# uni-medical/UniMedVL

Measured on AMD Instinct MI355X. Metric: VQA greedy decode tokens/s, UniMedVL-14B (BAGEL-7B-MoT dims), batch 8 x 448x448 per GPU, higher is better.
Workload: dtype bf16; 1 GPU; configs[1]: UniMedVL-14B bf16 VQA greedy decode, batch=8 448x448, 1xMI355X; batch_per_gpu=8, image=448x448, parallelism=dp1, decode=hipGraph

## Files before the change

include/unimedvl_hip.h:

```cpp
#ifndef UNIMEDVL_HIP_H
#define UNIMEDVL_HIP_H
#include <stddef.h>
#include <stdint.h>

#ifdef __cplusplus
extern "C" {
#endif

typedef void* umv_stream_t;

int umv_version(void);
const char* umv_last_error(void);

size_t umv_packed_weight_elems(int N, int K);
int umv_pack_weight_bf16(const uint16_t* w, uint16_t* packed, int N, int K, umv_stream_t stream);
size_t umv_repacked_weight_elems(int N, int K, int th);
int umv_repack_weight_rows_bf16(const uint16_t* packed16, uint16_t* out, int N, int K, int th, umv_stream_t stream);
int umv_pack_weight_swiglu_bf16(const uint16_t* gate, const uint16_t* up, uint16_t* packed, int I, int K,
                                umv_stream_t stream);

enum {
    UMV_EPI_BIAS = 1,
    UMV_EPI_GELU_TANH = 2,
    UMV_EPI_SILU = 4,
// ... 26 lines not shown
    const int64_t* sample_step;
} umv_gemm_args;
int umv_gemm_bf16(const umv_gemm_args* a, umv_stream_t stream);
int umv_gemm_tile_config(int M, int N, int K);

size_t umv_packed_weight_fp8_bytes(int N, int K);
int umv_quantize_pack_weight_fp8(const uint16_t* w, const uint16_t* w_up, uint8_t* packed8, float* scale, uint16_t* deq,
                                 uint16_t* deq_up, int rows, int K, umv_stream_t stream);
int umv_gemm_fp8w(const umv_gemm_args* a, umv_stream_t stream);

size_t umv_packed_weight_mxfp4_bytes(int N, int K);
int umv_quantize_pack_weight_mxfp4(const uint16_t* w, const uint16_t* w_up, uint8_t* packed4, uint16_t* deq, uint16_t* deq_up,
                                   int rows, int K, umv_stream_t stream);
int umv_gemm_mxfp4w(const umv_gemm_args* a, umv_stream_t stream);
int umv_gemm_mxfp4t(const umv_gemm_args* a, umv_stream_t stream);

size_t umv_packed_weight_fp8_mfma_bytes(int N, int K);
int umv_repack_weight_fp8_mfma(const uint8_t* packed8, uint8_t* out, int N, int K, umv_stream_t stream);
int umv_quantize_act_fp8(const uint16_t* x, int64_t ldx, const int32_t* row_idx, uint8_t* xq, int64_t ldq, float* x_scale,
                         uint16_t* deq, int64_t ldd, int M, int K, umv_stream_t stream);
typedef struct {
    const uint8_t* xq;
    int64_t ldq;
    const float* x_scale;
    const uint8_t* wp;
    const float* w_scale;
    const uint16_t* bias;
    const uint16_t* residual;
    int64_t ldr;
    void* out;
// ... 118 lines not shown
```

unimedvl_amd/_lib.py:

```python
import ctypes as C
import os

HERE = os.path.dirname(os.path.abspath(__file__))
LIB_PATH = os.environ.get("UMV_LIB_PATH") or os.path.join(HERE, "lib", "libunimedvl_hip.so")

EPI_BIAS, EPI_GELU_TANH, EPI_SILU, EPI_RESIDUAL, EPI_SWIGLU, EPI_OUT_F32 = 1, 2, 4, 8, 16, 32


class GemmArgs(C.Structure):
    _fields_ = [
        ("x", C.c_void_p), ("ldx", C.c_int64), ("wp", C.c_void_p), ("bias", C.c_void_p),
        ("residual", C.c_void_p), ("ldr", C.c_int64), ("out", C.c_void_p), ("ldo", C.c_int64),
        ("row_idx", C.c_void_p), ("M", C.c_int), ("N", C.c_int), ("K", C.c_int), ("epilogue", C.c_int),
        ("norm_w", C.c_void_p), ("norm_eps", C.c_float), ("tile_rows", C.c_int), ("w_scale", C.c_void_p),
        ("k_splits", C.c_int), ("split_stride", C.c_int64), ("argmax_partial", C.c_void_p), ("x_rows", C.c_int64),
        ("sample_temperature", C.c_float), ("sample_seed", C.c_uint64), ("sample_step", C.c_void_p),
    ]


class QkvPostArgs(C.Structure):
    _fields_ = [
        ("qkv", C.c_void_p), ("q_out", C.c_void_p), ("k_slab", C.c_void_p), ("vt_slab", C.c_void_p),
        ("k_seg_stride", C.c_int64), ("k_head_stride", C.c_int64), ("v_seg_stride", C.c_int64),
        ("v_head_stride", C.c_int64), ("v_d_stride", C.c_int64),
# ... 44 lines not shown
    "umv_last_error": (C.c_char_p, []),
    "umv_packed_weight_elems": (C.c_size_t, [C.c_int, C.c_int]),
    "umv_pack_weight_bf16": (C.c_int, [C.c_void_p, C.c_void_p, C.c_int, C.c_int, C.c_void_p]),
    "umv_repacked_weight_elems": (C.c_size_t, [C.c_int, C.c_int, C.c_int]),
    "umv_repack_weight_rows_bf16": (C.c_int, [C.c_void_p, C.c_void_p, C.c_int, C.c_int, C.c_int, C.c_void_p]),
    "umv_pack_weight_swiglu_bf16": (C.c_int, [C.c_void_p, C.c_void_p, C.c_void_p, C.c_int, C.c_int, C.c_void_p]),
    "umv_gemm_bf16": (C.c_int, [C.POINTER(GemmArgs), C.c_void_p]),
    "umv_packed_weight_fp8_bytes": (C.c_size_t, [C.c_int, C.c_int]),
    "umv_quantize_pack_weight_fp8": (C.c_int, [C.c_void_p, C.c_void_p, C.c_void_p, C.c_void_p, C.c_void_p, C.c_void_p,
                                               C.c_int, C.c_int, C.c_void_p]),
    "umv_gemm_fp8w": (C.c_int, [C.POINTER(GemmArgs), C.c_void_p]),
    "umv_packed_weight_mxfp4_bytes": (C.c_size_t, [C.c_int, C.c_int]),
    "umv_quantize_pack_weight_mxfp4": (C.c_int, [C.c_void_p, C.c_void_p, C.c_void_p, C.c_void_p, C.c_void_p, C.c_int, C.c_int,
                                                 C.c_void_p]),
    "umv_gemm_mxfp4w": (C.c_int, [C.POINTER(GemmArgs), C.c_void_p]),
    "umv_gemm_mxfp4t": (C.c_int, [C.POINTER(GemmArgs), C.c_void_p]),
    "umv_residual_rmsnorm_bf16": (C.c_int, [C.c_void_p, C.c_int, C.c_int64, C.c_int64, C.c_void_p, C.c_void_p, C.c_void_p, C.c_int,
                                            C.c_int, C.c_float, C.c_void_p]),
    "umv_rmsnorm_bf16": (C.c_int, [C.c_void_p, C.c_void_p, C.c_void_p, C.c_void_p, C.c_void_p, C.c_int, C.c_int,
                                   C.c_float, C.c_void_p]),
    "umv_layernorm_bf16": (C.c_int, [C.c_void_p, C.c_void_p, C.c_void_p, C.c_void_p, C.c_int, C.c_int, C.c_float,
                                     C.c_void_p]),
    "umv_embed_gather_bf16": (C.c_int, [C.c_void_p, C.c_void_p, C.c_void_p, C.c_void_p, C.c_int, C.c_int, C.c_void_p]),
    "umv_add_rows_bf16": (C.c_int, [C.c_void_p, C.c_void_p, C.c_void_p, C.c_void_p, C.c_void_p, C.c_void_p, C.c_int,
                                    C.c_int, C.c_void_p]),
    "umv_argmax_bf16": (C.c_int, [C.c_void_p, C.c_int64, C.c_void_p, C.c_int, C.c_int, C.c_void_p]),
    "umv_sample_bf16": (C.c_int, [C.c_void_p, C.c_int64, C.c_void_p, C.c_int, C.c_int, C.c_float, C.c_uint64, C.c_void_p,
                                  C.c_void_p]),
    "umv_cast_pad_f32_bf16": (C.c_int, [C.c_void_p, C.c_int64, C.c_void_p, C.c_int64, C.c_int, C.c_int, C.c_int,
                                        C.c_void_p]),
# ... 62 lines not shown
```

unimedvl_amd/build.py:

```python
import hashlib
import os
import subprocess
import sys

HERE = os.path.dirname(os.path.abspath(__file__))
CSRC = os.path.join(HERE, "csrc")
LIBDIR = os.path.join(HERE, "lib")
LIB = os.path.join(LIBDIR, "libunimedvl_hip.so")
SOURCES = ["host_error.hip", "elementwise.hip", "pack.hip", "gemm.hip", "gemm_w4.hip", "gemm_fp8mfma.hip", "gemm_mxfp4.hip", "gemm_mxfp4t.hip", "attention.hip", "attention_prefill.hip", "vision.hip"]
FLAGS = ["--offload-arch=gfx950", "-O3", "-std=c++17", "-fPIC", "-ffp-contract=off",
         "-Wno-unused-result", "-fgpu-rdc" if False else "-fno-gpu-rdc"]
FILE_FLAGS = {"attention_prefill.hip": ["-mllvm", "-amdgpu-mfma-vgpr-form"]}
if os.environ.get("UMV_ATTN_TRACE", "0") not in ("0", ""):
    FILE_FLAGS["attention_prefill.hip"] = FILE_FLAGS["attention_prefill.hip"] + ["-DUMV_ATTN_TRACE"]
if os.environ.get("UMV_ATTN_PAIR_DEBUG", "0") not in ("0", ""):
    FILE_FLAGS["attention_prefill.hip"] = FILE_FLAGS["attention_prefill.hip"] + ["-DUMV_ATTN_PAIR_DEBUG=1"]
if os.environ.get("UMV_GEMM_ABLATIONS", "0") not in ("0", ""):
    FILE_FLAGS["gemm_w4.hip"] = ["-DUMV_GEMM_ABLATIONS"]


def _stamp():
    h = hashlib.sha256()
    for f in sorted(os.listdir(CSRC)) + ["../../include/unimedvl_hip.h"]:
        p = os.path.join(CSRC, f)
# ... 59 lines not shown
```

unimedvl_amd/config.py:

```python
import json
import os
from dataclasses import dataclass, field, asdict
from typing import Tuple


@dataclass
class UniMedVLConfig:
    hidden: int = 3584
    layers: int = 28
    heads: int = 28
    kv_heads: int = 4
    inter: int = 18944
    vocab: int = 152064
    rope_theta: float = 1e6
    rms_eps: float = 1e-6
    max_position: int = 32768
    llm_weight_dtype: str = "bf16"
    llm_fp4_keep_bf16: bool = True
    llm_act_dtype: str = "bf16"
    vit_hidden: int = 1152
    vit_layers: int = 26
    vit_heads: int = 16
    vit_inter: int = 4304
    patch: int = 14
    vit_side: int = 70
    ln_eps: float = 1e-6
    max_latent: int = 64
    latent_patch: int = 2
    z_channels: int = 16
    vae_ch: int = 128
    vae_mult: Tuple[int, ...] = (1, 2, 4, 4)
    vae_res: int = 2
    scale_factor: float = 0.3611
# ... 42 lines not shown
```

unimedvl_amd/csrc/gemm_skinny.h:

```cpp
#pragma once
#include "common.h"
#include "../../include/unimedvl_hip.h"
#include "gemm_epilogue.h"
#include "gemm_internal.h"
#include "quant.h"

#define SK_WAVES 8
#define SK_XMAX 16

template <int NT_>
struct SkBf16 {
    static constexpr int NT = NT_, KH = 1;
    struct Unit { bf16x8 w[NT]; };
    int TH, tile_elems;
    bool rowlane;
    const bf16_t* wbase[NT];
    __device__ __forceinline__ SkBf16(const umv_gemm_args& a, int KT, int NTT, int, int nt0, int lane) {
        const int r = lane & 15, g = lane >> 4;
        TH = a.tile_rows > 0 ? a.tile_rows : 16;
        tile_elems = 4 * TH * 8;
        rowlane = r < TH;
#pragma unroll
        for (int t = 0; t < NT; ++t) {
            const bool tv = (nt0 + t) < NTT;
            wbase[t] = a.wp + ((int64_t)(tv ? nt0 + t : 0) * KT) * tile_elems + (g * TH + (rowlane ? r : 0)) * 8;
        }
    }
    __device__ __forceinline__ void load(Unit& b, int kt, bool ok) const {
#pragma unroll
        for (int t = 0; t < NT; ++t)
            b.w[t] = (ok && rowlane) ? __builtin_nontemporal_load(reinterpret_cast<const bf16x8*>(wbase[t] + (int64_t)kt * tile_elems)) : zero_frag();
    }
    __device__ __forceinline__ void frags(const Unit& b, bf16x8 (&wf)[KH][NT]) const {
#pragma unroll
        for (int t = 0; t < NT; ++t) wf[0][t] = b.w[t];
    }
};

template <int NT_>
struct SkE4m3 {
    static constexpr int NT = NT_, KH = 2, TH = 16;
    struct Unit { u32x4 w[NT]; };
    const uint8_t* wbase[NT];
    float wscale[NT];
    __device__ __forceinline__ SkE4m3(const umv_gemm_args& a, int KT8, int NTT, int, int nt0, int lane) {
        const uint8_t* wq = reinterpret_cast<const uint8_t*>(a.wp);
#pragma unroll
        for (int t = 0; t < NT; ++t) {
            const bool tv = (nt0 + t) < NTT;
            const int nt = tv ? nt0 + t : 0;
            wbase[t] = wq + ((int64_t)nt * KT8 * 64 + lane) * 16;
            wscale[t] = a.w_scale[nt * 16 + (lane & 15)];
        }
    }
    __device__ __forceinline__ void load(Unit& b, int kt, bool ok) const {
#pragma unroll
        for (int t = 0; t < NT; ++t)
            b.w[t] = ok ? __builtin_nontemporal_load(reinterpret_cast<const u32x4*>(wbase[t] + (int64_t)kt * 1024)) : (u32x4){0u, 0u, 0u, 0u};
    }
    __device__ __forceinline__ void frags(const Unit& b, bf16x8 (&wf)[KH][NT]) const {
#pragma unroll
        for (int t = 0; t < NT; ++t) cvt_fp8x16(b.w[t], wscale[t], wf[0][t], wf[1][t]);
    }
};

template <int NP>
struct SkMxfp4 {
    static constexpr int NT = 2 * NP, KH = 2, TH = 16;
    struct Unit { u32x4 w[NP]; uint32_t s[NP]; };
    const uint8_t* wbase[NP];
    const uint8_t* sbase[NP];
    __device__ __forceinline__ SkMxfp4(const umv_gemm_args& a, int KT8, int, int NPT, int, int lane) {
        const uint8_t* img = reinterpret_cast<const uint8_t*>(a.wp);
        const uint8_t* scales = img + (int64_t)NPT * KT8 * 1024;
        const int p0 = blockIdx.x * NP;
#pragma unroll
        for (int i = 0; i < NP; ++i) {
            const int p = (p0 + i) < NPT ? p0 + i : 0;
            wbase[i] = img + ((int64_t)p * KT8 * 64 + lane) * 16;
            sbase[i] = scales + ((int64_t)p * KT8 * 16 + (lane & 15)) * 4;
        }
    }
    __device__ __forceinline__ void load(Unit& b, int kt, bool ok) const {
#pragma unroll
        for (int i = 0; i < NP; ++i) {
            b.w[i] = ok ? __builtin_nontemporal_load(reinterpret_cast<const u32x4*>(wbase[i] + (int64_t)kt * 1024)) : (u32x4){0u, 0u, 0u, 0u};
            b.s[i] = ok ? *reinterpret_cast<const uint32_t*>(sbase[i] + (int64_t)kt * 64) : 0x7F7F7F7Fu;
        }
    }
    __device__ __forceinline__ void frags(const Unit& b, bf16x8 (&wf)[KH][NT]) const {
#pragma unroll
        for (int i = 0; i < NP; ++i) {
            const uint32_t s = b.s[i];
            wf[0][2 * i] = cvt_fp4x8(b.w[i].x, e8m0_scale(s & 0xFFu));
            wf[1][2 * i] = cvt_fp4x8(b.w[i].y, e8m0_scale((s >> 8) & 0xFFu));
            wf[0][2 * i + 1] = cvt_fp4x8(b.w[i].z, e8m0_scale((s >> 16) & 0xFFu));
            wf[1][2 * i + 1] = cvt_fp4x8(b.w[i].w, e8m0_scale(s >> 24));
        }
    }
};

template <int NW, int NT, int MB>
__device__ __forceinline__ void skinny16_reduce_epilogue(const umv_gemm_args& a, float* red, const f32x4 (&acc)[NT][MB], int tid,
                                                         int lane, int wave, int nt0, int NTT, int nsplit, int TH) {
    constexpr int E4 = NT * MB;
#pragma unroll
    for (int t = 0; t < NT; ++t)
#pragma unroll
        for (int mb = 0; mb < MB; ++mb) reinterpret_cast<f32x4*>(red)[(wave * E4 + t * MB + mb) * 64 + lane] = acc[t][mb];
    __syncthreads();
    EpiCtx e{a.bias, a.residual, a.ldr, a.out, a.ldo, a.N, a.epilogue};
    if (nsplit > 1) {
// ... 65 lines not shown
    bool xvalid[MB];
#pragma unroll
    for (int mb = 0; mb < MB; ++mb) {
        int m = mb * 16 + r;
        xvalid[mb] = m < a.M;
        int64_t row = xvalid[mb] ? (a.row_idx ? (int64_t)a.row_idx[m] : (int64_t)m) : 0;
        xrow[mb] = a.x + row * a.ldx;
    }
    f32x4 acc[NT][MB];
#pragma unroll
    for (int t = 0; t < NT; ++t)
#pragma unroll
        for (int mb = 0; mb < MB; ++mb) acc[t][mb] = (f32x4){0.f, 0.f, 0.f, 0.f};

    const int nsplit = a.k_splits > 1 ? a.k_splits : 1;
    const int kts = (KT + nsplit - 1) / nsplit;
    const int ks0 = (int)blockIdx.y * kts, ks1 = min(KT, ks0 + kts);
    const int kt_per = (max(0, ks1 - ks0) + SK_WAVES - 1) / SK_WAVES;
    const int kt_begin = ks0 + wave * kt_per;
    const int kt_end = min(ks1, kt_begin + kt_per);
    constexpr int UPL = 2 / KH;
    const int kt_lo = XL != 0 ? (kt_begin & -UPL) : kt_begin;
    const int nk = max(0, kt_end - kt_lo);
    const int nchunks = (nk + U - 1) / U;
    const F f(a, KT, NTT, NPT, nt0, lane);
    static_assert(!XL || ((U * KH) % 2 == 0 && NORM == 0), "full-line x staging: whole lines per chunk, no fused norm");
    static_assert(XL != 1 || MB == 1, "one-piece staging serves one 16-row tile of at most 8 valid rows");
    constexpr int XLN = U * KH / 2, XLP = XL == 1 ? 1 : 2 * MB;
    const int xchunk = (lane & 7) ^ ((lane >> 3) & 7);
    const bf16_t* xprow[XL ? XLP : 1];
    bool xpvalid[XL ? XLP : 1];
    if constexpr (XL != 0) {
#pragma unroll
        for (int q = 0; q < XLP; ++q) {
            const int m = q * 8 + (lane >> 3);
            xpvalid[q] = m < a.M;
            const int64_t row = xpvalid[q] ? (a.row_idx ? (int64_t)a.row_idx[m] : (int64_t)m) : 0;
            xprow[q] = a.x + row * a.ldx + xchunk * 8;
        }
    }
    char* xstage = reinterpret_cast<char*>(red) + wave * (XLN * XLP * 1024);
// ... 106 lines not shown
                const int rr = XL == 1 ? (r & 7) : r;
#pragma unroll
                for (int u = 0; u < U; ++u)
#pragma unroll
                    for (int h = 0; h < KH; ++h)
#pragma unroll
                        for (int mb = 0; mb < MB; ++mb) {
                            const int j = u * KH + h;
                            b.x[u][h][mb] = *reinterpret_cast<const bf16x8*>(xstage + (j >> 1) * (XLP * 1024) + (mb * 16 + rr) * 128 +
                                                                             ((((j & 1) * 4 + g) ^ (rr & 7)) << 4));
                        }
            }
#pragma unroll
            for (int u = 0; u < U; ++u) {
                bf16x8 wf[KH][NT];
                f.frags(b.w[u], wf);
#pragma unroll
                for (int h = 0; h < KH; ++h)
#pragma unroll
                    for (int t = 0; t < NT; ++t)
#pragma unroll
                        for (int mb = 0; mb < MB; ++mb) acc[t][mb] = mfma16(wf[h][t], b.x[u][h][mb], acc[t][mb]);
            }
        }
    };
    for (int c = 0; c < nchunks; c += 2) {
        if (DB && c + 1 < nchunks) load_chunk(c + 1, b1);
        consume(b0, c);
        if (c + 1 < nchunks) {
            if (!DB) load_chunk(c + 1, b1);
            if (c + 2 < nchunks && DB) load_chunk(c + 2, b0);
// ... 42 lines not shown
```

unimedvl_amd/csrc/pack.hip:

```cpp
#include "common.h"
#include "../../include/unimedvl_hip.h"
#include "quant.h"
#include <stdlib.h>

__global__ void pack_weight_kernel(const bf16_t* __restrict__ w, bf16_t* __restrict__ p, int N, int K, int NTT,
                                   int KT, int interleave_I, const bf16_t* __restrict__ w2) {
    int64_t gid = (int64_t)blockIdx.x * blockDim.x + threadIdx.x;
    int64_t total = (int64_t)NTT * KT * 64;
    if (gid >= total) return;
    int lane = (int)(gid & 63);
    int64_t tile = gid >> 6;
    int kt = (int)(tile % KT);
    int nt = (int)(tile / KT);
    int r = lane & 15, g = lane >> 4;
    int k = kt * 32 + g * 8;
    const bf16_t* src = w;
    int n;
    if (interleave_I > 0) {
        int t = nt >> 1;
        n = t * 16 + r;
        src = (nt & 1) ? w2 : w;
        if (n >= interleave_I) n = -1;
    } else {
        n = nt * 16 + r;
// ... 262 lines not shown
                                              uint16_t* deq_up, int rows, int K, umv_stream_t stream) {
    UMV_CHECK(w && packed4 && rows > 0 && K > 0, UMV_ERR_ARG, "quantize_pack_weight_mxfp4: bad args");
    UMV_CHECK((K % 32) == 0 && K <= 65536, UMV_ERR_ARG, "quantize_pack_weight_mxfp4: K (%d) must be a multiple of 32 (the block) and <= 65536",
              K);
    UMV_CHECK(!w_up || (rows % 16) == 0, UMV_ERR_ARG, "quantize_pack_weight_mxfp4: SwiGLU image needs I %% 16 == 0 (I=%d)", rows);
    UMV_CHECK(!(deq_up && !w_up), UMV_ERR_ARG, "quantize_pack_weight_mxfp4: deq_up without w_up");
    UMV_CHECK(((uintptr_t)w | (uintptr_t)w_up | (uintptr_t)deq | (uintptr_t)deq_up | (uintptr_t)packed4) % 16 == 0, UMV_ERR_ARG,
              "quantize_pack_weight_mxfp4: every buffer must be 16-byte aligned");
    const int NTT = (w_up ? 2 : 1) * ((rows + 15) / 16), NP = (NTT + 1) / 2, KT8 = (K + 63) / 64;
    const size_t lds = (size_t)32 * 2 * KT8;
    hipLaunchKernelGGL(quantize_pack_mxfp4_kernel, dim3(NP), dim3(256), lds, (hipStream_t)stream, (const bf16_t*)w, (const bf16_t*)w_up,
                       packed4, (bf16_t*)deq, (bf16_t*)deq_up, rows, K, KT8, NTT, NP);
    UMV_LAUNCH_CHECK();
    return UMV_OK;
}
```

unimedvl_amd/ops.py:

```python
import ctypes as C
import functools

import torch

from . import _lib
from ._lib import (EPI_BIAS, EPI_GELU_TANH, EPI_OUT_F32, EPI_RESIDUAL, EPI_SILU, EPI_SWIGLU, AttnArgs, GemmArgs,
                   QkvPostArgs, check)

BF16 = torch.bfloat16


_raw_stream = getattr(torch._C, "_cuda_getCurrentRawStream", None)


def _stream():
    if _raw_stream is not None:
        return C.c_void_p(_raw_stream(torch.cuda.current_device()))
    return C.c_void_p(torch.cuda.current_stream().cuda_stream)


def on_device(fn):
    @functools.wraps(fn)
    def wrapper(self, *args, **kwargs):
        dev = torch.device(self.device)
# ... 12 lines not shown
    return torch.cuda.device(dev)


def _p(t):
    return None if t is None else C.c_void_p(t.data_ptr())


def _req(t, dtype, name):
    if not t.is_cuda:
        raise _lib.UmvError(f"{name}: tensor must live on the GPU (no CPU fallback)")
    if t.dtype != dtype:
        raise _lib.UmvError(f"{name}: expected {dtype}, got {t.dtype}")
    return t


class PackedLinear:

    __slots__ = ("wp", "bias", "N", "K", "swiglu", "th", "w8", "scale", "w8m", "w4")

    def __init__(self, wp, bias, N, K, swiglu=False, th=16, w8=None, scale=None, w4=None):
        self.wp, self.bias, self.N, self.K, self.swiglu, self.th = wp, bias, N, K, swiglu, th
        self.w8, self.scale = w8, scale
        self.w8m = None
        self.w4 = w4

    def drop_bf16(self):
        if self.w4 is None:
            raise _lib.UmvError("drop_bf16 needs MXFP4 weights (from_weight_mxfp4 / from_gate_up_mxfp4)")
        self.wp = None
        return self

    def enable_fp8_mfma(self, keep_bf16=False):
        if self.w8m is not None:
            if not keep_bf16:
                self.wp = None
            return self
        if self.w8 is None:
            raise _lib.UmvError("enable_fp8_mfma needs fp8 weights (from_weight_fp8 / from_gate_up_fp8)")
        lib = _lib.load()
# ... 94 lines not shown
    @staticmethod
    def from_gate_up(gate, up):
        lib = _lib.load()
        gate = _req(gate.contiguous(), BF16, "gate")
        up = _req(up.contiguous(), BF16, "up")
        I, K = gate.shape
        assert I % 16 == 0, "intermediate size must be a multiple of 16"
        wp = torch.empty(lib.umv_packed_weight_elems(2 * I, K), dtype=BF16, device=gate.device)
        check(lib.umv_pack_weight_swiglu_bf16(_p(gate), _p(up), _p(wp), I, K, _stream()), "umv_pack_weight_swiglu_bf16")
        return PackedLinear(wp, None, 2 * I, K, swiglu=True)

    def nbytes(self):
        return self.wp.numel() * 2 if self.wp is not None else self.w4.numel()


def gemm(x, lin, out=None, *, M=None, residual=None, act=None, row_idx=None, out_f32=False, use_bias=True,
         norm_w=None, norm_eps=1e-6, act8=False, argmax_partial=None, sample=None):
    lib = _lib.load()
    _req(x, BF16, "x")
    assert x.stride(-1) == 1
    M = x.shape[0] if M is None else M
    flags = 0
    if lin.bias is not None and use_bias:
        flags |= EPI_BIAS
    if act == "gelu_tanh":
        flags |= EPI_GELU_TANH
    elif act == "silu":
        flags |= EPI_SILU
    elif act is not None:
        raise ValueError(act)
    if lin.swiglu:
        flags |= EPI_SWIGLU
# ... 66 lines not shown
            row_idx=row_idx.data_ptr() if row_idx is not None else None,
            M=M, N=lin.N, K=lin.K, epilogue=flags, norm_w=None, norm_eps=norm_eps, tile_rows=0,
            w_scale=lin.scale.data_ptr(), argmax_partial=amax, **_sample_fields(sample, amax))
        check(lib.umv_gemm_fp8w(C.byref(a), _stream()), "umv_gemm_fp8w")
        return out
    a = GemmArgs(
        x=x.data_ptr(), ldx=x.stride(0), wp=lin.wp.data_ptr(),
        bias=lin.bias.data_ptr() if (flags & EPI_BIAS) else None,
        residual=residual.data_ptr() if residual is not None else None,
        ldr=residual.stride(0) if residual is not None else 0,
        out=out.data_ptr(), ldo=out.stride(0),
        row_idx=row_idx.data_ptr() if row_idx is not None else None,
        M=M, N=lin.N, K=lin.K, epilogue=flags,
        norm_w=norm_w.data_ptr() if norm_w is not None else None, norm_eps=norm_eps, tile_rows=lin.th, argmax_partial=amax,
        x_rows=x.shape[0], **_sample_fields(sample, amax))
    check(lib.umv_gemm_bf16(C.byref(a), _stream()), "umv_gemm_bf16")
    return out


def rmsnorm(x, w, eps, out=None, w_gen=None, expert=None):
    lib = _lib.load()
    _req(x, BF16, "x")
    T, H = x.shape
    out = torch.empty_like(x) if out is None else out
    check(lib.umv_rmsnorm_bf16(_p(x), _p(w), _p(w_gen), _p(expert), _p(out), T, H, eps, _stream()), "umv_rmsnorm_bf16")
    return out


def layernorm(x, w, b, eps, out=None):
    lib = _lib.load()
# ... 134 lines not shown
          "umv_quantize_act_fp8")
    return out


def _sample_fields(sample, amax):
    if sample is None:
        return {}
    if amax is None:
        raise _lib.UmvError("gemm: sample=(temperature, seed, step) is a mode of the argmax_partial epilogue")
    t, seed, step = sample
    if not float(t) > 0.0:
        raise _lib.UmvError(f"gemm: sampling temperature must be > 0 (got {t})")
    return dict(sample_temperature=float(t), sample_seed=int(seed) & (2 ** 64 - 1), sample_step=None if step is None else step.data_ptr())


def gemm_splitk(x, lin, partials, k_splits, *, M=None):
    lib = _lib.load()
    _req(x, BF16, "x")
    _req(partials, torch.float32, "partials")
    M = x.shape[0] if M is None else M
    assert partials.dim() == 3 and partials.shape[0] == k_splits and partials.shape[2] == lin.N and partials.is_contiguous()
    assert lin.th == 16 and not lin.swiglu
    a = GemmArgs(x=x.data_ptr(), ldx=x.stride(0), wp=None if lin.wp is None else lin.wp.data_ptr(), out=partials.data_ptr(), ldo=lin.N,
                 M=M, N=lin.N, K=lin.K, epilogue=0, tile_rows=0, k_splits=k_splits, split_stride=partials.stride(0))
    if lin.w8 is not None:
        a.wp, a.w_scale = lin.w8.data_ptr(), lin.scale.data_ptr()
        check(lib.umv_gemm_fp8w(C.byref(a), _stream()), "umv_gemm_fp8w")
    elif lin.w4 is not None and M <= 64:
        a.wp = lin.w4.data_ptr()
        check(lib.umv_gemm_mxfp4w(C.byref(a), _stream()), "umv_gemm_mxfp4w")
    elif lin.w4 is not None and lin.wp is None:
        a.wp = lin.w4.data_ptr()
        check(lib.umv_gemm_mxfp4t(C.byref(a), _stream()), "umv_gemm_mxfp4t")
    else:
        check(lib.umv_gemm_bf16(C.byref(a), _stream()), "umv_gemm_bf16")
    return partials


def residual_rmsnorm(partials, seq, w, eps, out):
    lib = _lib.load()
    _req(partials, torch.float32, "partials")
    _req(seq, BF16, "seq")
    S, T, H = partials.shape
    assert seq.shape == (T, H) and seq.is_contiguous() and out.is_contiguous() and partials.is_contiguous()
    check(lib.umv_residual_rmsnorm_bf16(_p(partials), S, partials.stride(0), partials.stride(1), _p(seq), _p(w), _p(out), T, H, eps,
                                        _stream()), "umv_residual_rmsnorm_bf16")
    return out

# ... 115 lines not shown
```

unimedvl_amd/weights.py:

```python
import math

import torch

from . import ops
from .config import UniMedVLConfig

BF16 = torch.bfloat16


class LayerWeights:
    __slots__ = ("qkv", "o", "gate_up", "down", "in_norm", "post_norm", "q_norm", "k_norm")


def _dev(t, device):
    return t.to(device=device, dtype=BF16).contiguous()


class _NoStore:
    @staticmethod
    def linear(key, build):
        return build()

    @staticmethod
    def tensor(name, build):
# ... 37 lines not shown
        self.act8 = cfg.llm_act_dtype == "fp8"
        keep = self.fp4_keep_bf16 = bool(cfg.llm_fp4_keep_bf16) or not fp4
        self.embed = _tensor(get, device, p + "embed_tokens.weight")
        self.und, self.gen = [], []
        for l in range(cfg.layers):
            self.und.append(self._layer(get, device, p + f"layers.{l}.", "", fp8, fp4, keep))
            self.gen.append(self._layer(get, device, p + f"layers.{l}.", "_moe_gen", fp8, fp4, keep) if load_gen else None)
            if self.act8:
                for lw in (self.und[-1], self.gen[-1]):
                    if lw is not None:
                        for lin in (lw.qkv, lw.o, lw.gate_up, lw.down):
                            lin.enable_fp8_mfma()
        self.norm = _tensor(get, device, p + "norm.weight")
        self.norm_gen = _tensor(get, device, p + "norm_moe_gen.weight") if load_gen else None
        self.lm_head = _linear(get, device, "language_model.lm_head.weight", fp8=fp8 or fp4)
        hd = cfg.head_dim
        inv_freq = 1.0 / (cfg.rope_theta ** (torch.arange(0, hd, 2, dtype=torch.int64).float() / hd))
        pos = torch.arange(cfg.max_position, dtype=torch.float32)
        freqs = (inv_freq[None, :, None].float() @ pos[None, None, :]).transpose(1, 2)[0]
        emb = torch.cat((freqs, freqs), dim=-1)
        self.cos = emb.cos().to(BF16).to(device)
        self.sin = emb.sin().to(BF16).to(device)

    @staticmethod
    def _layer(get, device, p, suf, fp8=False, fp4=False, keep_bf16=True):
        lw = LayerWeights()
        a = p + "self_attn."
        st = _store(get)

        def build_qkv():
# ... 8 lines not shown
            u = _dev(get(p + f"mlp{suf}.up_proj.weight"), device)
            if fp4:
                return ops.PackedLinear.from_gate_up_mxfp4(g, u, keep_bf16=keep_bf16)
            return ops.PackedLinear.from_gate_up_fp8(g, u) if fp8 else ops.PackedLinear.from_gate_up(g, u)
        lw.qkv = st.linear(a + f"qkv_proj{suf}", build_qkv)
        lw.o = _linear(get, device, a + f"o_proj{suf}.weight", fp8=fp8, fp4=fp4, keep_bf16=keep_bf16)
        lw.gate_up = st.linear(p + f"mlp{suf}.gate_up_proj", build_gate_up)
        lw.down = _linear(get, device, p + f"mlp{suf}.down_proj.weight", fp8=fp8, fp4=fp4, keep_bf16=keep_bf16)
        lw.in_norm = _tensor(get, device, p + f"input_layernorm{suf}.weight")
        lw.post_norm = _tensor(get, device, p + f"post_attention_layernorm{suf}.weight")
        lw.q_norm = _tensor(get, device, a + f"q_norm{suf}.weight")
        lw.k_norm = _tensor(get, device, a + f"k_norm{suf}.weight")
        return lw

    def decode_weight_bytes(self):
        nb = (lambda lin: lin.w8.numel()) if self.fp8 else (lambda lin: lin.w4.numel()) if self.fp4 else (lambda lin: lin.nbytes())
        n = self.lm_head.w8.numel() if self.fp4 else nb(self.lm_head)
        for lw in self.und:
            n += nb(lw.qkv) + nb(lw.o) + nb(lw.gate_up) + nb(lw.down)
        return n


class ViTLayer:
    __slots__ = ("qkv", "out", "fc1", "fc2", "ln1_w", "ln1_b", "ln2_w", "ln2_b")


class ViTWeights:
    def __init__(self, cfg: UniMedVLConfig, get, device):
        p = "vit_model.vision_model."
        self.k_in = 3 * cfg.patch ** 2
        self.k_pad = (self.k_in + 31) // 32 * 32
# ... 71 lines not shown
```

Baseline: 2550 tokens/s.

## Stream losslessly 13-bit-compressed bf16 weights in decode MLP and lm_head GEMMs

```diff
diff --git a/include/unimedvl_hip.h b/include/unimedvl_hip.h
--- a/include/unimedvl_hip.h
+++ b/include/unimedvl_hip.h
@@ -64,6 +64,10 @@
                                    int rows, int K, umv_stream_t stream);
 int umv_gemm_mxfp4w(const umv_gemm_args* a, umv_stream_t stream);
 int umv_gemm_mxfp4t(const umv_gemm_args* a, umv_stream_t stream);
+
+size_t umv_packed_weight_z13_bytes(int N, int K);
+int umv_pack_weight_z13(const uint16_t* packed16, uint8_t* z13, int N, int K, umv_stream_t stream);
+int umv_gemm_z13w(const umv_gemm_args* a, const void* z13, umv_stream_t stream);
 
 size_t umv_packed_weight_fp8_mfma_bytes(int N, int K);
 int umv_repack_weight_fp8_mfma(const uint8_t* packed8, uint8_t* out, int N, int K, umv_stream_t stream);
diff --git a/unimedvl_amd/_lib.py b/unimedvl_amd/_lib.py
--- a/unimedvl_amd/_lib.py
+++ b/unimedvl_amd/_lib.py
@@ -82,6 +82,9 @@
     "umv_quantize_pack_weight_mxfp4": (C.c_int, [C.c_void_p, C.c_void_p, C.c_void_p, C.c_void_p, C.c_void_p, C.c_int, C.c_int,
                                                  C.c_void_p]),
     "umv_gemm_mxfp4w": (C.c_int, [C.POINTER(GemmArgs), C.c_void_p]),
+    "umv_packed_weight_z13_bytes": (C.c_size_t, [C.c_int, C.c_int]),
+    "umv_pack_weight_z13": (C.c_int, [C.c_void_p, C.c_void_p, C.c_int, C.c_int, C.c_void_p]),
+    "umv_gemm_z13w": (C.c_int, [C.POINTER(GemmArgs), C.c_void_p, C.c_void_p]),
     "umv_gemm_mxfp4t": (C.c_int, [C.POINTER(GemmArgs), C.c_void_p]),
     "umv_residual_rmsnorm_bf16": (C.c_int, [C.c_void_p, C.c_int, C.c_int64, C.c_int64, C.c_void_p, C.c_void_p, C.c_void_p, C.c_int,
                                             C.c_int, C.c_float, C.c_void_p]),
diff --git a/unimedvl_amd/build.py b/unimedvl_amd/build.py
--- a/unimedvl_amd/build.py
+++ b/unimedvl_amd/build.py
@@ -7,7 +7,7 @@
 CSRC = os.path.join(HERE, "csrc")
 LIBDIR = os.path.join(HERE, "lib")
 LIB = os.path.join(LIBDIR, "libunimedvl_hip.so")
-SOURCES = ["host_error.hip", "elementwise.hip", "pack.hip", "gemm.hip", "gemm_w4.hip", "gemm_fp8mfma.hip", "gemm_mxfp4.hip", "gemm_mxfp4t.hip", "attention.hip", "attention_prefill.hip", "vision.hip"]
+SOURCES = ["host_error.hip", "elementwise.hip", "pack.hip", "gemm.hip", "gemm_w4.hip", "gemm_fp8mfma.hip", "gemm_mxfp4.hip", "gemm_mxfp4t.hip", "gemm_z13.hip", "attention.hip", "attention_prefill.hip", "vision.hip"]
 FLAGS = ["--offload-arch=gfx950", "-O3", "-std=c++17", "-fPIC", "-ffp-contract=off",
          "-Wno-unused-result", "-fgpu-rdc" if False else "-fno-gpu-rdc"]
 FILE_FLAGS = {"attention_prefill.hip": ["-mllvm", "-amdgpu-mfma-vgpr-form"]}
diff --git a/unimedvl_amd/config.py b/unimedvl_amd/config.py
--- a/unimedvl_amd/config.py
+++ b/unimedvl_amd/config.py
@@ -17,6 +17,7 @@
     max_position: int = 32768
     llm_weight_dtype: str = "bf16"
     llm_fp4_keep_bf16: bool = True
+    llm_decode_z13: bool = True
     llm_act_dtype: str = "bf16"
     vit_hidden: int = 1152
     vit_layers: int = 26
diff --git a/unimedvl_amd/csrc/gemm_skinny.h b/unimedvl_amd/csrc/gemm_skinny.h
--- a/unimedvl_amd/csrc/gemm_skinny.h
+++ b/unimedvl_amd/csrc/gemm_skinny.h
@@ -11,6 +11,7 @@
 template <int NT_>
 struct SkBf16 {
     static constexpr int NT = NT_, KH = 1;
+    static constexpr bool HALVES = false;
     struct Unit { bf16x8 w[NT]; };
     int TH, tile_elems;
     bool rowlane;
@@ -40,6 +41,7 @@
 template <int NT_>
 struct SkE4m3 {
     static constexpr int NT = NT_, KH = 2, TH = 16;
+    static constexpr bool HALVES = false;
     struct Unit { u32x4 w[NT]; };
     const uint8_t* wbase[NT];
     float wscale[NT];
@@ -67,6 +69,7 @@
 template <int NP>
 struct SkMxfp4 {
     static constexpr int NT = 2 * NP, KH = 2, TH = 16;
+    static constexpr bool HALVES = false;
     struct Unit { u32x4 w[NP]; uint32_t s[NP]; };
     const uint8_t* wbase[NP];
     const uint8_t* sbase[NP];
@@ -96,6 +99,83 @@
             wf[1][2 * i] = cvt_fp4x8(b.w[i].y, e8m0_scale((s >> 8) & 0xFFu));
             wf[0][2 * i + 1] = cvt_fp4x8(b.w[i].z, e8m0_scale((s >> 16) & 0xFFu));
             wf[1][2 * i + 1] = cvt_fp4x8(b.w[i].w, e8m0_scale(s >> 24));
+        }
+    }
+};
+
+typedef __attribute__((ext_vector_type(2))) unsigned short umv_u16x2;
+__device__ __forceinline__ uint32_t z13_pk_mad(uint32_t q, uint32_t mul, uint32_t add) {
+    const umv_u16x2 r = __builtin_bit_cast(umv_u16x2, q) * __builtin_bit_cast(umv_u16x2, mul) + __builtin_bit_cast(umv_u16x2, add);
+    return __builtin_bit_cast(uint32_t, r);
+}
+__device__ __forceinline__ uint32_t z13_pk_shr8(uint32_t q) {
+    const umv_u16x2 r = __builtin_bit_cast(umv_u16x2, q) >> (umv_u16x2){8, 8};
+    return __builtin_bit_cast(uint32_t, r);
+}
+template <int E>
+__device__ __forceinline__ bf16x8 z13_frag(uint32_t sm0, uint32_t sm1, uint32_t n, uint32_t t, uint32_t mul, uint32_t base7, uint32_t emask) {
+    constexpr int EA = 2 * E, EB = 2 * E + 1;
+    const uint32_t ta = EA < 4 ? t << (4 - EA) : t >> (EA - 4), tb = EB < 4 ? t << (4 - EB) : t >> (EB - 4);
+    const uint32_t qa = (ta & 0x10101010u) | (n & 0x0F0F0F0Fu), qb = (tb & 0x10101010u) | ((n >> 4) & 0x0F0F0F0Fu);
+    const uint32_t e[4] = {z13_pk_mad(qa, mul, base7), z13_pk_mad(z13_pk_shr8(qa), mul, base7), z13_pk_mad(qb, mul, base7),
+                           z13_pk_mad(z13_pk_shr8(qb), mul, base7)};
+    const uint32_t p[4] = {__builtin_amdgcn_perm(sm0, sm0, 0x01010000u), __builtin_amdgcn_perm(sm0, sm0, 0x03030202u),
+                           __builtin_amdgcn_perm(sm1, sm1, 0x01010000u), __builtin_amdgcn_perm(sm1, sm1, 0x03030202u)};
+    u32x4 o;
+    o.x = (e[0] & emask) | (p[0] & ~emask);
+    o.y = (e[1] & emask) | (p[1] & ~emask);
+    o.z = (e[2] & emask) | (p[2] & ~emask);
+    o.w = (e[3] & emask) | (p[3] & ~emask);
+    return __builtin_bit_cast(bf16x8, o);
+}
+
+#define Z13_RECORD 3328
+__host__ __device__ __forceinline__ int64_t z13_head_bytes(int NPT) { return ((int64_t)NPT * 16 + 255) / 256 * 256; }
+
+template <int NP>
+struct SkZ13 {
+    static constexpr int NT = 2 * NP, KH = 2, TH = 16;
+    static constexpr bool HALVES = true;
+    struct Unit { u32x4 sm[NP][2]; u32x4 n[NP]; uint32_t t[NP]; };
+    const uint8_t* rec[NP];
+    uint32_t base7[NP];
+    uint32_t lane16, lane4;
+    __device__ __forceinline__ SkZ13(const umv_gemm_args& a, int KT8, int, int NPT, int, int lane) {
+        const uint8_t* img = reinterpret_cast<const uint8_t*>(a.wp);
+        const int p0 = blockIdx.x * NP;
+#pragma unroll
+        for (int i = 0; i < NP; ++i) {
+            const int p = (p0 + i) < NPT ? p0 + i : 0;
+            rec[i] = img + z13_head_bytes(NPT) + (int64_t)p * KT8 * Z13_RECORD;
+            const uint32_t b = reinterpret_cast<const uint32_t*>(img)[4 * p + 2] & 0xFFu;
+            base7[i] = (b << 7) * 0x10001u;
+        }
+        lane16 = (uint32_t)lane * 16u;
+        lane4 = 3072u + (uint32_t)lane * 4u;
+    }
+    __device__ __forceinline__ void load(Unit& b, int kt, bool ok) const {
+        const int ktu = __builtin_amdgcn_readfirstlane(kt);
+#pragma unroll
+        for (int i = 0; i < NP; ++i) {
+            const uint8_t* r = rec[i] + (int64_t)ktu * Z13_RECORD;
+            const u32x4 z = {0u, 0u, 0u, 0u};
+            b.sm[i][0] = ok ? __builtin_nontemporal_load(reinterpret_cast<const u32x4*>(r + lane16)) : z;
+            b.sm[i][1] = ok ? __builtin_nontemporal_load(reinterpret_cast<const u32x4*>(r + 1024 + lane16)) : z;
+            b.n[i] = ok ? __builtin_nontemporal_load(reinterpret_cast<const u32x4*>(r + 2048 + lane16)) : z;
+            b.t[i] = ok ? __builtin_nontemporal_load(reinterpret_cast<const uint32_t*>(r + lane4)) : 0u;
+        }
+    }
+    __device__ __forceinline__ void frags(const Unit& b, bf16x8 (&wf)[KH][NT], bool in0, bool in1) const {
+        const bool v0 = __builtin_amdgcn_readfirstlane((int)in0) != 0, v1 = __builtin_amdgcn_readfirstlane((int)in1) != 0;
+#pragma unroll
+        for (int i = 0; i < NP; ++i) {
+            const uint32_t mul0 = v0 ? 0xFF80FF80u : 0u, mul1 = v1 ? 0xFF80FF80u : 0u;
+            const uint32_t b0 = v0 ? base7[i] : 0u, b1 = v1 ? base7[i] : 0u;
+            const uint32_t m0 = v0 ? 0x7F807F80u : 0xFFFFFFFFu, m1 = v1 ? 0x7F807F80u : 0xFFFFFFFFu;
+            wf[0][2 * i] = z13_frag<0>(b.sm[i][0].x, b.sm[i][0].y, b.n[i].x, b.t[i], mul0, b0, m0);
+            wf[1][2 * i] = z13_frag<1>(b.sm[i][0].z, b.sm[i][0].w, b.n[i].y, b.t[i], mul1, b1, m1);
+            wf[0][2 * i + 1] = z13_frag<2>(b.sm[i][1].x, b.sm[i][1].y, b.n[i].z, b.t[i], mul0, b0, m0);
+            wf[1][2 * i + 1] = z13_frag<3>(b.sm[i][1].z, b.sm[i][1].w, b.n[i].w, b.t[i], mul1, b1, m1);
         }
     }
 };
@@ -191,17 +271,22 @@
         for (int mb = 0; mb < MB; ++mb) acc[t][mb] = (f32x4){0.f, 0.f, 0.f, 0.f};
 
     const int nsplit = a.k_splits > 1 ? a.k_splits : 1;
-    const int kts = (KT + nsplit - 1) / nsplit;
-    const int ks0 = (int)blockIdx.y * kts, ks1 = min(KT, ks0 + kts);
+    constexpr int SG = F::HALVES ? KH : 1;
+    const int KTG = KT * SG;
+    const int kts = (KTG + nsplit - 1) / nsplit;
+    const int ks0 = (int)blockIdx.y * kts, ks1 = min(KTG, ks0 + kts);
     const int kt_per = (max(0, ks1 - ks0) + SK_WAVES - 1) / SK_WAVES;
-    const int kt_begin = ks0 + wave * kt_per;
-    const int kt_end = min(ks1, kt_begin + kt_per);
+    const int g_begin = ks0 + wave * kt_per;
+    const int g_end = min(ks1, g_begin + kt_per);
+    const int kt_begin = g_begin / SG;
+    const int kt_end = g_end > g_begin ? (g_end + SG - 1) / SG : kt_begin;
     constexpr int UPL = 2 / KH;
     const int kt_lo = XL != 0 ? (kt_begin & -UPL) : kt_begin;
     const int nk = max(0, kt_end - kt_lo);
     const int nchunks = (nk + U - 1) / U;
     const F f(a, KT, NTT, NPT, nt0, lane);
     static_assert(!XL || ((U * KH) % 2 == 0 && NORM == 0), "full-line x staging: whole lines per chunk, no fused norm");
+    static_assert(!F::HALVES || NORM == 0, "half-unit slices: no fused norm");
     static_assert(XL != 1 || MB == 1, "one-piece staging serves one 16-row tile of at most 8 valid rows");
     constexpr int XLN = U * KH / 2, XLP = XL == 1 ? 1 : 2 * MB;
     const int xchunk = (lane & 7) ^ ((lane >> 3) & 7);
@@ -338,7 +423,12 @@
 #pragma unroll
             for (int u = 0; u < U; ++u) {
                 bf16x8 wf[KH][NT];
-                f.frags(b.w[u], wf);
+                if constexpr (F::HALVES) {
+                    const int g0 = (kt_lo + c * U + u) * SG;
+                    f.frags(b.w[u], wf, g0 >= g_begin && g0 < g_end, g0 + 1 >= g_begin && g0 + 1 < g_end);
+                } else {
+                    f.frags(b.w[u], wf);
+                }
 #pragma unroll
                 for (int h = 0; h < KH; ++h)
 #pragma unroll
diff --git a/unimedvl_amd/csrc/gemm_z13.hip b/unimedvl_amd/csrc/gemm_z13.hip
--- /dev/null
+++ b/unimedvl_amd/csrc/gemm_z13.hip
@@ -0,0 +1,65 @@
+#include "common.h"
+#include "../../include/unimedvl_hip.h"
+#include "gemm_skinny.h"
+
+template <int MB, int NP, int U, int XL = 0>
+__global__ __launch_bounds__(SK_WAVES * 64) void gemm_skinny13_kernel(umv_gemm_args a, const uint8_t* z13, int KT8, int NTT, int NPT) {
+    const int KT = 2 * KT8, nsplit = a.k_splits > 1 ? a.k_splits : 1;
+    const int kts = (KT + nsplit - 1) / nsplit;
+    const int ks0 = (int)blockIdx.y * kts, ks1 = min(KT, ks0 + kts);
+    uint64_t any = 0;
+    if (ks1 > ks0) {
+        const int b0 = ks0 >> 4, b1 = (ks1 + 15) >> 4;
+        const uint64_t range = (b1 - b0 >= 64 ? ~0ull : ((1ull << (b1 - b0)) - 1ull)) << b0;
+        const uint64_t* flags = reinterpret_cast<const uint64_t*>(z13);
+#pragma unroll
+        for (int i = 0; i < NP; ++i) {
+            const int p = (int)blockIdx.x * NP + i;
+            if (p < NPT) any |= flags[2 * p] & range;
+        }
+    }
+    if (any != 0) {
+        gemm_skinny_body<SkBf16<2 * NP>, MB, 2 * U, true, 0, XL>(a, KT, NTT, 0);
+    } else {
+        a.wp = reinterpret_cast<const uint16_t*>(z13);
+        gemm_skinny_body<SkZ13<NP>, MB, U, true, 0, XL>(a, KT8, NTT, NPT);
+    }
+}
+
+template <int MB, int NP, int U>
+static int launch_skinny13(const umv_gemm_args& a, const uint8_t* z13, int KT8, int NTT, int NPT, hipStream_t s) {
+    return launch_skinny_body<MB, 2 * NP, U, 2, 0>([](auto XL) { return &gemm_skinny13_kernel<MB, NP, U, decltype(XL)::value>; }, a, KT8,
+                                                   NTT, s, z13, KT8, NTT, NPT);
+}
+
+extern "C" int umv_gemm_z13w(const umv_gemm_args* ap, const void* z13, umv_stream_t stream) {
+    UMV_CHECK(ap != nullptr, UMV_ERR_ARG, "gemm_z13w: null args");
+    umv_gemm_args a = *ap;
+    UMV_CHECK(a.x && a.wp && a.out && z13, UMV_ERR_ARG, "gemm_z13w: null pointer (x, wp = the bf16 image, out and z13 are required)");
+    UMV_CHECK(!a.w_scale, UMV_ERR_ARG, "gemm_z13w: w_scale must be NULL");
+    if (const int rc = umv_gemm_check_args(a, "gemm_z13w", 32)) return rc;
+    UMV_CHECK((a.K % 64) == 0 && a.K <= 32768, UMV_ERR_UNSUPPORTED, "gemm_z13w: K (%d) must be a multiple of 64 and <= 32768", a.K);
+    UMV_CHECK(a.M <= 64, UMV_ERR_UNSUPPORTED, "gemm_z13w: the 13-bit image is the decode (M <= 64) layout; use umv_gemm_bf16 for M=%d", a.M);
+    UMV_CHECK(!a.norm_w && (a.tile_rows == 0 || a.tile_rows == 16), UMV_ERR_UNSUPPORTED, "gemm_z13w: no fused norm / th-row tiles");
+    UMV_CHECK(a.k_splits <= 1 || (!(a.epilogue & UMV_EPI_SWIGLU) && a.split_stride > 0 && a.k_splits <= 64), UMV_ERR_UNSUPPORTED,
+              "gemm_z13w: split-K (k_splits=%d) needs no SwiGLU, split_stride > 0, k_splits <= 64", a.k_splits);
+    UMV_CHECK(!a.argmax_partial || (a.k_splits <= 1 && !a.row_idx && !(a.epilogue & (UMV_EPI_SWIGLU | UMV_EPI_OUT_F32))), UMV_ERR_UNSUPPORTED,
+              "gemm_z13w: argmax_partial needs bf16 out, no SwiGLU / split-K / row_idx");
+    UMV_CHECK(a.sample_temperature >= 0.f && (a.sample_temperature == 0.f || a.argmax_partial), UMV_ERR_ARG,
+              "gemm_z13w: sample_temperature (%g) is a mode of the argmax_partial epilogue and must be >= 0", (double)a.sample_temperature);
+    UMV_CHECK(((uintptr_t)z13 % 256) == 0, UMV_ERR_ARG, "gemm_z13w: the 13-bit image must be 256-byte aligned");
+    if (a.M == 0) return UMV_OK;
+    hipStream_t s = (hipStream_t)stream;
+    const uint8_t* z = reinterpret_cast<const uint8_t*>(z13);
+    const int KT8 = a.K / 64, NTT = (a.N + 15) / 16, NPT = (NTT + 1) / 2;
+    if (a.k_splits > 1) {
+        if (a.M <= 16) return launch_skinny13<1, 2, 1>(a, z, KT8, NTT, NPT, s);
+        if (a.M <= 32) return launch_skinny13<2, 2, 1>(a, z, KT8, NTT, NPT, s);
+        return launch_skinny13<4, 1, 1>(a, z, KT8, NTT, NPT, s);
+    }
+    const bool two = (a.epilogue & UMV_EPI_SWIGLU) || NTT >= 1024;
+    if (a.M <= 16) return launch_skinny13<1, 1, 2>(a, z, KT8, NTT, NPT, s);
+    if (a.M <= 32) return two ? launch_skinny13<2, 2, 1>(a, z, KT8, NTT, NPT, s) : launch_skinny13<2, 1, 2>(a, z, KT8, NTT, NPT, s);
+    if (two && !a.argmax_partial && a.K >= 1024) return umv_gemm_bf16(&a, stream);
+    return launch_skinny13<4, 1, 1>(a, z, KT8, NTT, NPT, s);
+}
diff --git a/unimedvl_amd/csrc/pack.hip b/unimedvl_amd/csrc/pack.hip
--- a/unimedvl_amd/csrc/pack.hip
+++ b/unimedvl_amd/csrc/pack.hip
@@ -300,3 +300,105 @@
     UMV_LAUNCH_CHECK();
     return UMV_OK;
 }
+
+#define Z13_RECORD 3328
+static inline size_t z13_head_bytes_host(size_t NPT) { return (NPT * 16 + 255) / 256 * 256; }
+
+__global__ __launch_bounds__(256) void z13_base_kernel(const bf16_t* __restrict__ p16, unsigned long long* __restrict__ head, int N, int KT,
+                                                       int NTT) {
+    __shared__ uint32_t smax[256];
+    const int p = blockIdx.x, tid = threadIdx.x;
+    uint32_t m = 0;
+    for (int tt = 0; tt < 2; ++tt) {
+        const int nt = 2 * p + tt;
+        if (nt >= NTT) continue;
+        for (int64_t idx = tid; idx < (int64_t)KT * 64; idx += 256) {
+            const int lane = (int)(idx & 63);
+            if (nt * 16 + (lane & 15) >= N) continue;
+            const u32x4 v = *reinterpret_cast<const u32x4*>(p16 + ((int64_t)nt * KT * 64 + idx) * 8);
+            const uint32_t wd[4] = {v.x, v.y, v.z, v.w};
+#pragma unroll
+            for (int j = 0; j < 4; ++j) {
+                const uint32_t f0 = (wd[j] >> 7) & 0xFFu, f1 = (wd[j] >> 23) & 0xFFu;
+                if (f0 != 255u) m = max(m, f0);
+                if (f1 != 255u) m = max(m, f1);
+            }
+        }
+    }
+    smax[tid] = m;
+    __syncthreads();
+    for (int s = 128; s > 0; s >>= 1) {
+        if (tid < s) smax[tid] = max(smax[tid], smax[tid + s]);
+        __syncthreads();
+    }
+    if (tid == 0) {
+        head[2 * p] = 0;
+        head[2 * p + 1] = smax[0];
+    }
+}
+
+__global__ __launch_bounds__(256) void z13_encode_kernel(const bf16_t* __restrict__ p16, uint8_t* __restrict__ img, int N, int KT8, int NTT,
+                                                         int NPT, int64_t total) {
+    const int64_t gid = (int64_t)blockIdx.x * blockDim.x + threadIdx.x;
+    if (gid >= total) return;
+    const int lane = (int)(gid & 63);
+    const int u = (int)((gid >> 6) % KT8);
+    const int p = (int)((gid >> 6) / KT8);
+    const int KT = 2 * KT8;
+    const uint32_t base = img[(int64_t)p * 16 + 8];
+    uint32_t sm[2][4] = {{0u, 0u, 0u, 0u}, {0u, 0u, 0u, 0u}}, nib[4] = {0u, 0u, 0u, 0u}, top = 0u;
+    bool flag = false;
+#pragma unroll
+    for (int tt = 0; tt < 2; ++tt) {
+        const int nt = 2 * p + tt;
+        if (nt >= NTT) continue;
+        const bool counts = nt * 16 + (lane & 15) < N;
+#pragma unroll
+        for (int h = 0; h < 2; ++h) {
+            const u32x4 v = *reinterpret_cast<const u32x4*>(p16 + (((int64_t)nt * KT + 2 * u + h) * 64 + lane) * 8);
+            const uint32_t wd[4] = {v.x, v.y, v.z, v.w};
+            const int f = 2 * tt + h;
+#pragma unroll
+            for (int j = 0; j < 8; ++j) {
+                const uint32_t w = (wd[j >> 1] >> (16 * (j & 1))) & 0xFFFFu;
+                const uint32_t field = (w >> 7) & 0xFFu;
+                const bool codable = field != 255u && base >= field && base - field <= 30u;
+                const uint32_t code = codable ? base - field : 0u;
+                flag = flag || (counts && !codable);
+                const int byte = ((j & 1) << 1) | ((j >> 1) & 1), q = j >> 2;
+                sm[tt][2 * h + (j >> 2)] |= (((w >> 8) & 0x80u) | (w & 0x7Fu)) << (8 * (j & 3));
+                nib[f] |= (code & 15u) << (8 * byte + 4 * q);
+                top |= (code >> 4) << (8 * byte + 2 * f + q);
+            }
+        }
+    }
+    uint8_t* rec = img + ((int64_t)NPT * 16 + 255) / 256 * 256 + ((int64_t)p * KT8 + u) * Z13_RECORD;
+    *reinterpret_cast<u32x4*>(rec + lane * 16) = (u32x4){sm[0][0], sm[0][1], sm[0][2], sm[0][3]};
+    *reinterpret_cast<u32x4*>(rec + 1024 + lane * 16) = (u32x4){sm[1][0], sm[1][1], sm[1][2], sm[1][3]};
+    *reinterpret_cast<u32x4*>(rec + 2048 + lane * 16) = (u32x4){nib[0], nib[1], nib[2], nib[3]};
+    *reinterpret_cast<uint32_t*>(rec + 3072 + lane * 4) = top;
+    if (flag) atomicOr(reinterpret_cast<unsigned long long*>(img) + 2 * p, 1ull << (u >> 3));
+}
+
+extern "C" size_t umv_packed_weight_z13_bytes(int N, int K) {
+    if (N <= 0 || K <= 0) return 0;
+    const size_t np = ((size_t)(N + 15) / 16 + 1) / 2, kt8 = (size_t)(K + 63) / 64;
+    return z13_head_bytes_host(np) + np * kt8 * Z13_RECORD;
+}
+
+extern "C" int umv_pack_weight_z13(const uint16_t* packed16, uint8_t* z13, int N, int K, umv_stream_t stream) {
+    UMV_CHECK(packed16 && z13 && N > 0 && K > 0, UMV_ERR_ARG, "pack_weight_z13: bad args");
+    UMV_CHECK((K % 64) == 0 && K <= 32768, UMV_ERR_ARG, "pack_weight_z13: K (%d) must be a multiple of 64 and <= 32768", K);
+    UMV_CHECK(((uintptr_t)packed16 % 16) == 0 && ((uintptr_t)z13 % 256) == 0, UMV_ERR_ARG,
+              "pack_weight_z13: the bf16 image must be 16-byte and the 13-bit image 256-byte aligned");
+    const int NTT = (N + 15) / 16, NPT = (NTT + 1) / 2, KT8 = K / 64;
+    hipStream_t s = (hipStream_t)stream;
+    hipLaunchKernelGGL(z13_base_kernel, dim3(NPT), dim3(256), 0, s, (const bf16_t*)packed16,
+                       reinterpret_cast<unsigned long long*>(z13), N, 2 * KT8, NTT);
+    UMV_LAUNCH_CHECK();
+    const int64_t total = (int64_t)NPT * KT8 * 64;
+    hipLaunchKernelGGL(z13_encode_kernel, dim3((unsigned)((total + 255) / 256)), dim3(256), 0, s, (const bf16_t*)packed16, z13, N, KT8, NTT,
+                       NPT, total);
+    UMV_LAUNCH_CHECK();
+    return UMV_OK;
+}
diff --git a/unimedvl_amd/ops.py b/unimedvl_amd/ops.py
--- a/unimedvl_amd/ops.py
+++ b/unimedvl_amd/ops.py
@@ -50,15 +50,27 @@
     return t
 
 
+Z13_MAX_ROWS = 32
+
+
 class PackedLinear:
 
-    __slots__ = ("wp", "bias", "N", "K", "swiglu", "th", "w8", "scale", "w8m", "w4")
+    __slots__ = ("wp", "bias", "N", "K", "swiglu", "th", "w8", "scale", "w8m", "w4", "wz")
 
     def __init__(self, wp, bias, N, K, swiglu=False, th=16, w8=None, scale=None, w4=None):
         self.wp, self.bias, self.N, self.K, self.swiglu, self.th = wp, bias, N, K, swiglu, th
         self.w8, self.scale = w8, scale
         self.w8m = None
         self.w4 = w4
+        self.wz = None
+
+    def build_z13(self):
+        if self.wp is None or self.th != 16 or self.w8 is not None or self.w4 is not None or self.K % 64 or self.K > 32768:
+            raise _lib.UmvError("build_z13 needs a plain bf16 linear (16-row image) with K a multiple of 64, K <= 32768")
+        lib = _lib.load()
+        self.wz = torch.empty(lib.umv_packed_weight_z13_bytes(self.N, self.K), dtype=torch.uint8, device=self.wp.device)
+        check(lib.umv_pack_weight_z13(_p(self.wp), _p(self.wz), self.N, self.K, _stream()), "umv_pack_weight_z13")
+        return self
 
     def drop_bf16(self):
         if self.w4 is None:
@@ -183,8 +195,18 @@
         return self.wp.numel() * 2 if self.wp is not None else self.w4.numel()
 
 
+def _z13_takes(lin, M, z13, form):
+    if lin.wz is None or z13 is False:
+        return False
+    if z13:
+        return M <= 64
+    if form == "splitk":
+        return M <= Z13_MAX_ROWS
+    return form == "epilogue" and (M <= 8 or 16 < M <= Z13_MAX_ROWS)
+
+
 def gemm(x, lin, out=None, *, M=None, residual=None, act=None, row_idx=None, out_f32=False, use_bias=True,
-         norm_w=None, norm_eps=1e-6, act8=False, argmax_partial=None, sample=None):
+         norm_w=None, norm_eps=1e-6, act8=False, argmax_partial=None, sample=None, z13=None):
     lib = _lib.load()
     _req(x, BF16, "x")
     assert x.stride(-1) == 1
@@ -281,6 +303,10 @@
         M=M, N=lin.N, K=lin.K, epilogue=flags,
         norm_w=norm_w.data_ptr() if norm_w is not None else None, norm_eps=norm_eps, tile_rows=lin.th, argmax_partial=amax,
         x_rows=x.shape[0], **_sample_fields(sample, amax))
+    if _z13_takes(lin, M, z13, "epilogue" if (lin.swiglu or amax is not None) else None) and norm_w is None and \
+            not (flags & (EPI_GELU_TANH | EPI_SILU)):
+        check(lib.umv_gemm_z13w(C.byref(a), lin.wz.data_ptr(), _stream()), "umv_gemm_z13w")
+        return out
     check(lib.umv_gemm_bf16(C.byref(a), _stream()), "umv_gemm_bf16")
     return out
 
@@ -445,7 +471,7 @@
     return dict(sample_temperature=float(t), sample_seed=int(seed) & (2 ** 64 - 1), sample_step=None if step is None else step.data_ptr())
 
 
-def gemm_splitk(x, lin, partials, k_splits, *, M=None):
+def gemm_splitk(x, lin, partials, k_splits, *, M=None, z13=None):
     lib = _lib.load()
     _req(x, BF16, "x")
     _req(partials, torch.float32, "partials")
@@ -463,6 +489,8 @@
     elif lin.w4 is not None and lin.wp is None:
         a.wp = lin.w4.data_ptr()
         check(lib.umv_gemm_mxfp4t(C.byref(a), _stream()), "umv_gemm_mxfp4t")
+    elif _z13_takes(lin, M, z13, "splitk"):
+        check(lib.umv_gemm_z13w(C.byref(a), lin.wz.data_ptr(), _stream()), "umv_gemm_z13w")
     else:
         check(lib.umv_gemm_bf16(C.byref(a), _stream()), "umv_gemm_bf16")
     return partials
diff --git a/unimedvl_amd/weights.py b/unimedvl_amd/weights.py
--- a/unimedvl_amd/weights.py
+++ b/unimedvl_amd/weights.py
@@ -1,4 +1,6 @@
 import math
+import os
+import warnings
 
 import torch
 
@@ -75,6 +77,14 @@
         self.norm = _tensor(get, device, p + "norm.weight")
         self.norm_gen = _tensor(get, device, p + "norm_moe_gen.weight") if load_gen else None
         self.lm_head = _linear(get, device, "language_model.lm_head.weight", fp8=fp8 or fp4)
+        self.z13 = bool(cfg.llm_decode_z13) and not fp8 and not fp4 and os.environ.get("UMV_DECODE_Z13", "1") != "0"
+        if self.z13:
+            for lin in [self.lm_head] + [l for lw in self.und for l in (lw.gate_up, lw.down)]:
+                if lin.K % 64 == 0 and lin.K <= 32768 and lin.th == 16:
+                    lin.build_z13()
+                else:
+                    warnings.warn(f"llm_decode_z13: no 13-bit image for a {lin.N} x {lin.K} linear (needs K % 64 == 0, K <= 32768, "
+                                  "16-row tiles); its decode GEMMs stream the bf16 image")
         hd = cfg.head_dim
         inv_freq = 1.0 / (cfg.rope_theta ** (torch.arange(0, hd, 2, dtype=torch.int64).float() / hd))
         pos = torch.arange(cfg.max_position, dtype=torch.float32)
@@ -113,7 +123,8 @@
         return lw
 
     def decode_weight_bytes(self):
-        nb = (lambda lin: lin.w8.numel()) if self.fp8 else (lambda lin: lin.w4.numel()) if self.fp4 else (lambda lin: lin.nbytes())
+        bf16 = lambda lin: lin.wz.numel() if lin.wz is not None else lin.nbytes()
+        nb = (lambda lin: lin.w8.numel()) if self.fp8 else (lambda lin: lin.w4.numel()) if self.fp4 else bf16
         n = self.lm_head.w8.numel() if self.fp4 else nb(self.lm_head)
         for lw in self.und:
             n += nb(lw.qkv) + nb(lw.o) + nb(lw.gate_up) + nb(lw.down)
```

After: 2692 tokens/s, median of 6. 1.06x the previous value.
